# mj129/Tramba

Measured on AMD Instinct MI355X. Metric: images/sec fwd Tramba-V 384x384, higher is better.
Workload: dtype bf16; 1 GPU; Tramba-V (VMamba-B encoder) 384x384 bf16 inference, batch 4 per GPU, random-init weights (seed 1026), randn images; global_batch=4, launch=hipGraph replay, decoder guide branches on a side stream

## Files before the change

include/tramba_hip.h:

```cpp
#ifndef TRAMBA_HIP_H
#define TRAMBA_HIP_H

#include <stddef.h>
#include <stdint.h>

#ifdef __cplusplus
extern "C" {
#endif

typedef enum { TRAMBA_F32 = 0, TRAMBA_F16 = 1, TRAMBA_BF16 = 2 } tramba_dtype;

typedef enum {
    TRAMBA_SCAN_RASTER = 0,
    TRAMBA_SCAN_LINE = 1,
    TRAMBA_SCAN_HELIX = 2,
    TRAMBA_SCAN_WINDOW = 3,
    TRAMBA_SCAN_DILATION = 4
} tramba_scan_family;

typedef enum { TRAMBA_ACT_NONE = 0, TRAMBA_ACT_SILU = 1, TRAMBA_ACT_GELU = 2,
               TRAMBA_ACT_SIGMOID_GATE = 3 ,
               TRAMBA_ACT_GELU_GRAD_MUL = 4
             } tramba_act;

// ... 6 lines not shown
int tramba_abi_version(void);
int tramba_device_error(void);
int tramba_profile_enable(int which, int enable);
int tramba_profile_read(int which, double *total_ms, double *total_bytes);
int tramba_profile_min_units(int which, double min_units);
int tramba_tune_set(int knob, int value);
int tramba_tune_get(int knob);
#define TRAMBA_TUNE_MERGE_FORM 0
#define TRAMBA_TUNE_SCAN_FORM 1
#define TRAMBA_TUNE_SCAN_W 2
#define TRAMBA_TUNE_GEMM_TILE 3
#define TRAMBA_TUNE_MAILBOX_SKIP 4
#define TRAMBA_TUNE_DW_FORM 6
#define TRAMBA_TUNE_DW_ROWS 7
#define TRAMBA_TUNE_MERGE_PW 8
#define TRAMBA_TUNE_COUNT 9
#define TRAMBA_PROF_SCAN_BOUNDARY 0
#define TRAMBA_PROF_SCAN_FUSED 1
#define TRAMBA_PROF_GEMM 2
#define TRAMBA_PROF_MERGE 3
#define TRAMBA_PROF_SCAN_BWD 4
#define TRAMBA_PROF_WGRAD 5
#define TRAMBA_PROF_LAYERNORM 6
#define TRAMBA_PROF_DW 7
#define TRAMBA_PROF_COUNT 8

int tramba_scan_family_k(int family);
int tramba_default_window(int h);
int tramba_scan_table(int family, int h, int w, int param, int32_t *out);
int tramba_scan_table_inverse(const int32_t *table, int k, int l, int32_t *inv_ptr, int32_t *inv_idx);

// ... 115 lines not shown
int tramba_slab_sum(const float *part, float *out, int64_t n, int nslab, void *stream);
int tramba_multi_sum_strided(const float *const *parts, float *const *outs, const int64_t *n, const int64_t *stride,
                             const int *nslab, int count, void *stream);
int tramba_multi_sum(const float *const *parts, float *const *outs, const int64_t *n, const int *nslab, int count,
                     void *stream);

int tramba_expand_norm_head_cl(const void *x, const void *w, const float *ln_w, const float *ln_b,
                               const float *head_w, float head_b, float *y, int batch, int h, int wd, int cin, int p,
                               float eps, int dtype, void *stream);

int tramba_conv3x3s2_cl(const void *x, const void *w, const float *bias, void *y, int batch, int hin,
                        int win, int cin, int cout, int dtype, void *stream);
int tramba_stem_conv_ln_gelu(const void *img, const float *w, const float *bias, const float *ln_w,
                             const float *ln_b, void *y, int batch, int h, int wd, float eps,
                             int img_dtype, int dtype, void *stream);

#define TRAMBA_EVAL_NINT 520
#define TRAMBA_EVAL_NDBL 48
int tramba_saliency_stats(const float *pred, const unsigned char *gt, long long *ints, double *dbl, int batch, int h,
                          int w, void *stream);
#define TRAMBA_WFM_MAX_DIM 4096
int tramba_feature_transform(const unsigned char *gt, int *idx, int *dist2, int batch, int h, int w, void *stream);
size_t tramba_weighted_f_workspace(int batch, int h, int w);
int tramba_weighted_f_sums(const float *pred, const unsigned char *gt, const int *idx, const int *dist2, const double *gauss,
                           double *sums, void *workspace, size_t workspace_bytes, int batch, int h, int w, void *stream);

#define TRAMBA_FRAME_MAX_DIM 16384
#define TRAMBA_FRAME_MAX_OUT 2048
size_t tramba_resize_table_words(int in_h, int in_w, int out_h, int out_w);
int tramba_resize_table(int in_h, int in_w, int out_h, int out_w, const double *mean, const double *std, int *table,
// ... 120 lines not shown
```

tramba_amd/csrc/linear.hip:

```cpp
#include <stdlib.h>
#include <string.h>

#include <type_traits>

#include "common.h"

namespace tramba {

typedef __attribute__((ext_vector_type(8))) short frag8_t;
typedef __attribute__((ext_vector_type(8))) _Float16 frag8h_t;
typedef __attribute__((ext_vector_type(16))) float acc16_t;

template <typename T> struct Mfma;
template <> struct Mfma<__hip_bfloat16> {
    static constexpr int KSTEP = 16;
    using frag = frag8_t;
    static __device__ __forceinline__ acc16_t run(frag a, frag b, acc16_t c)
    {
        typedef __attribute__((ext_vector_type(8))) __bf16 bf8;
        return __builtin_amdgcn_mfma_f32_32x32x16_bf16(__builtin_bit_cast(bf8, a), __builtin_bit_cast(bf8, b), c, 0, 0, 0);
    }
};
template <> struct Mfma<__half> {
    static constexpr int KSTEP = 16;
// ... 567 lines not shown
    }
    for (; kt0 + NS <= nk; kt0 += NS) {
#pragma unroll
        for (int ui = 0; ui < NS; ++ui) kstep(kt0 + ui, ui & 1, pipe[ui % NS], pipe[(ui + 1) % NS]);
    }
#pragma unroll
    for (int ui = 0; ui < NS - 1; ++ui)
        if (kt0 + ui < nk) kstep(kt0 + ui, ui & 1, pipe[ui % NS], pipe[(ui + 1) % NS]);

    if constexpr (LNHEAD) {
        static_assert(BN == 128, "one tile = whole 128-channel groups");
        tile_epilogue_ln_head<T, BM>(acc, lds, hd, M, m0, n0);
    } else {
        tile_epilogue<T, TO, BM, BN>(acc, lds, bias, res, y, M, N, act, m0, n0);
    }
}

#define TRAMBA_DSR128_(OUT, ADDR, OFF) asm volatile("ds_read_b128 %0, %1 offset:" #OFF : "=v"(OUT) : "v"(ADDR) : "memory")

template <typename T, typename TO, int NSTG, bool LNIN = false, bool DUAL = false>
__global__ __launch_bounds__(256) void linear_dma_kernel(const T *__restrict__ x, const T *__restrict__ w,
                                                        const float *__restrict__ bias, const T *__restrict__ res,
                                                        TO *__restrict__ y, long M, int N, int K, int act,
                                                        LnIn li = LnIn{nullptr, 0.f}, TO *__restrict__ y_pre = nullptr)
{
#if defined(__HIP_DEVICE_COMPILE__)
    constexpr int BM = 64, BN = 64;
    constexpr int TILE_BYTES = (BM + BN) * kBK * 2;
    constexpr int EPI_BYTES = BM * (BN + 4) * 4;
    constexpr int LDS_BYTES = NSTG * TILE_BYTES > EPI_BYTES ? NSTG * TILE_BYTES : EPI_BYTES;
// ... 1041 lines not shown
extern "C" int tramba_expand_norm_head_cl(const void *x, const void *w, const float *ln_w, const float *ln_b,
                                          const float *head_w, float head_b, float *y, int batch, int h, int wd, int cin,
                                          int p, float eps, int dtype, void *stream)
{
    TRAMBA_CHECK(x && w && ln_w && ln_b && head_w && y, "expand_norm_head_cl: null tensor");
    TRAMBA_CHECK(batch > 0 && h > 0 && wd > 0 && cin > 0 && p > 0, "expand_norm_head_cl: empty shape");
    TRAMBA_CHECK(dtype == TRAMBA_BF16 || dtype == TRAMBA_F16, "expand_norm_head_cl: 16-bit dtypes only");
    TRAMBA_CHECK(cin % 64 == 0, "expand_norm_head_cl: Cin=%d must be a multiple of 64", cin);
    TRAMBA_CHECK(aligned16(x) && aligned16(w), "expand_norm_head_cl: tensors must be 16-byte aligned");
    const long m = (long)batch * h * wd;
    const int n = p * p * 128;
    TRAMBA_CHECK(m < 2147483647L && (m + 63) / 64 <= 65535, "expand_norm_head_cl: too many pixels");
    hipStream_t s = (hipStream_t)stream;
    ProfScope prof(TRAMBA_PROF_GEMM, s, 2.0 * (double)m * n * cin);
    const LnHead hd{ln_w, ln_b, head_w, head_b, eps, h, wd, p, y};
    dim3 grid((unsigned)(n / 128), (unsigned)((m + 63) / 64)), block(256);
    if (dtype == TRAMBA_BF16) {
        using T = __hip_bfloat16;
        hipLaunchKernelGGL((linear_lean_kernel<T, T, 64, 128, 1, true>), grid, block, 0, s, (const T *)x, (const T *)w,
                           (const float *)nullptr, (const T *)nullptr, (T *)nullptr, m, n, cin, 0, (const T *)nullptr, 0, hd);
    } else {
        using T = __half;
        hipLaunchKernelGGL((linear_lean_kernel<T, T, 64, 128, 1, true>), grid, block, 0, s, (const T *)x, (const T *)w,
                           (const float *)nullptr, (const T *)nullptr, (T *)nullptr, m, n, cin, 0, (const T *)nullptr, 0, hd);
    }
    TRAMBA_LAUNCH_CHECK();
    return TRAMBA_OK;
}

extern "C" int tramba_conv3x3s2_cl(const void *x, const void *w, const float *bias, void *y, int batch, int hin,
// ... 43 lines not shown
```

tramba_amd/csrc/stem.hip:

```cpp
#include "common.h"

namespace tramba {

constexpr int kStemCout = 64, kStemTaps = 27;

template <typename TI, typename T>
__global__ __launch_bounds__(256) void stem_conv_ln_gelu_kernel(const TI *__restrict__ img, const float *__restrict__ w,
                                                               const float *__restrict__ bias,
                                                               const float *__restrict__ ln_w,
                                                               const float *__restrict__ ln_b, T *__restrict__ y,
                                                               int B, int H, int W, int Ho, int Wo, float eps)
{
    __shared__ __attribute__((aligned(16))) float wl[kStemTaps][kStemCout];
    for (int t = threadIdx.x; t < kStemTaps * kStemCout; t += blockDim.x) {
        const int co = t / kStemTaps, tap = t % kStemTaps;
        wl[tap][co] = w[t];
    }
    __syncthreads();
    const long pix = (long)blockIdx.x * 64 + (threadIdx.x >> 2);
    const int part = threadIdx.x & 3;
    const long npix = (long)B * Ho * Wo;
    const bool ok = pix < npix;
    const long pp = ok ? pix : npix - 1;
    const int wo = (int)(pp % Wo);
    const long t2 = pp / Wo;
    const int ho = (int)(t2 % Ho), b = (int)(t2 / Ho);

    float acc[16];
#pragma unroll
    for (int j = 0; j < 16; ++j) acc[j] = bias[part * 16 + j];
#pragma unroll 1
    for (int ci = 0; ci < 3; ++ci)
#pragma unroll 1
        for (int ky = 0; ky < 3; ++ky) {
            const int hy = 2 * ho + ky - 1;
#pragma unroll
            for (int kx = 0; kx < 3; ++kx) {
                const int wx = 2 * wo + kx - 1;
                float v = 0.f;
                if (hy >= 0 && hy < H && wx >= 0 && wx < W) v = Cvt<TI>::to_f(img[(((long)b * 3 + ci) * H + hy) * W + wx]);
                const float4 *wp = reinterpret_cast<const float4 *>(&wl[ci * 9 + ky * 3 + kx][part * 16]);
#pragma unroll
                for (int q = 0; q < 4; ++q) {
                    const float4 ww = wp[q];
                    acc[4 * q + 0] = fmaf(v, ww.x, acc[4 * q + 0]);
                    acc[4 * q + 1] = fmaf(v, ww.y, acc[4 * q + 1]);
                    acc[4 * q + 2] = fmaf(v, ww.z, acc[4 * q + 2]);
                    acc[4 * q + 3] = fmaf(v, ww.w, acc[4 * q + 3]);
                }
            }
        }
    float s = 0.f;
#pragma unroll
    for (int j = 0; j < 16; ++j) s += acc[j];
    s += __shfl_xor(s, 1, 4);
    s += __shfl_xor(s, 2, 4);
    const float mean = s * (1.f / kStemCout);
    float q2 = 0.f;
#pragma unroll
    for (int j = 0; j < 16; ++j) {
        const float d = acc[j] - mean;
        q2 = fmaf(d, d, q2);
    }
    q2 += __shfl_xor(q2, 1, 4);
    q2 += __shfl_xor(q2, 2, 4);
    const float rstd = rsqrtf(q2 * (1.f / kStemCout) + eps);
    if (!ok) return;
    T *yo = y + pix * kStemCout + part * 16;
#pragma unroll
    for (int h8 = 0; h8 < 2; ++h8) {
        float o[8];
#pragma unroll
        for (int j = 0; j < 8; ++j) {
            const int c = part * 16 + h8 * 8 + j;
            o[j] = geluf_((acc[h8 * 8 + j] - mean) * rstd * ln_w[c] + ln_b[c]);
        }
        store_pack<T, 8>(yo + h8 * 8, o);
    }
}

}

using namespace tramba;

extern "C" int tramba_stem_conv_ln_gelu(const void *img, const float *w, const float *bias, const float *ln_w,
                                        const float *ln_b, void *y, int batch, int h, int wd, float eps,
                                        int img_dtype, int dtype, void *stream)
{
    TRAMBA_CHECK(img && w && bias && ln_w && ln_b && y, "stem_conv_ln_gelu: null tensor");
    TRAMBA_CHECK(batch > 0 && h > 0 && wd > 0, "stem_conv_ln_gelu: empty shape");
    TRAMBA_CHECK(img_dtype == TRAMBA_F32 || img_dtype == dtype, "stem_conv_ln_gelu: image must be f32 or the activation dtype");
    TRAMBA_CHECK(aligned16(y), "stem_conv_ln_gelu: output must be 16-byte aligned");
    const int ho = (h + 1) / 2, wo = (wd + 1) / 2;
    const long npix = (long)batch * ho * wo;
    dim3 grid((unsigned)((npix + 63) / 64)), block(256);
    hipStream_t s = (hipStream_t)stream;
    TRAMBA_DISPATCH_DTYPE(dtype, T, {
        if (img_dtype == TRAMBA_F32 && dtype != TRAMBA_F32)
            hipLaunchKernelGGL((stem_conv_ln_gelu_kernel<float, T>), grid, block, 0, s, (const float *)img, w, bias, ln_w,
                               ln_b, (T *)y, batch, h, wd, ho, wo, eps);
        else
            hipLaunchKernelGGL((stem_conv_ln_gelu_kernel<T, T>), grid, block, 0, s, (const T *)img, w, bias, ln_w, ln_b,
                               (T *)y, batch, h, wd, ho, wo, eps);
    });
    TRAMBA_LAUNCH_CHECK();
    return TRAMBA_OK;
}
```

tramba_amd/hip.py:

```python
import ctypes
import os
import threading
import weakref

import numpy as np
import torch

_HERE = os.path.dirname(os.path.abspath(__file__))
LIB_PATH = os.path.join(_HERE, "_lib", "libtramba_hip.so")

F32, F16, BF16 = 0, 1, 2
ACT_NONE, ACT_SILU, ACT_GELU, ACT_SIGMOID_GATE, ACT_GELU_GRAD_MUL = 0, 1, 2, 3, 4
SCAN_RASTER, SCAN_LINE, SCAN_HELIX, SCAN_WINDOW, SCAN_DILATION = range(5)
FAMILY = {"raster": SCAN_RASTER, "line": SCAN_LINE, "helix": SCAN_HELIX, "window": SCAN_WINDOW,
          "dilation": SCAN_DILATION}
PROF_SCAN_BOUNDARY, PROF_SCAN_FUSED, PROF_GEMM, PROF_MERGE, PROF_SCAN_BWD, PROF_WGRAD, PROF_LAYERNORM, PROF_DW = 0, 1, 2, 3, 4, 5, 6, 7

_DT = {torch.float32: F32, torch.float16: F16, torch.bfloat16: BF16}

c_int, c_i64, c_f, c_vp = ctypes.c_int, ctypes.c_int64, ctypes.c_float, ctypes.c_void_p

SIGNATURES = {
    "tramba_last_error": (ctypes.c_char_p, []),
    "tramba_abi_version": (c_int, []),
# ... 72 lines not shown
    "tramba_linear_ln_cl": (c_int, [c_vp] * 6 + [c_i64, c_int, c_int, c_f, c_int, c_int, c_int, c_vp]),
    "tramba_linear2_cl": (c_int, [c_vp, c_vp, c_int] + [c_vp] * 4 + [c_i64, c_int, c_int, c_int, c_int, c_int, c_vp]),
    "tramba_wgrad_workspace": (ctypes.c_size_t, [c_i64, c_int, c_int, c_int, c_int]),
    "tramba_wgrad_cl": (c_int, [c_vp] * 4 + [ctypes.c_size_t, c_i64, c_int, c_int, c_int, c_int, c_i64, c_i64, c_int, c_i64,
                                             c_i64, c_int, c_int, c_int, c_vp]),
    "tramba_rows_gemm_cl": (c_int, [c_vp] * 3 + [c_int, c_i64, c_int, c_int, c_int, c_int, c_int, c_vp]),
    "tramba_shadow_cast_multi": (c_int, [c_vp, c_int, c_i64, c_int, c_vp]),
    "tramba_slab_sum": (c_int, [c_vp, c_vp, c_i64, c_int, c_vp]),
    "tramba_multi_sum": (c_int, [c_vp, c_vp, c_vp, c_vp, c_int, c_vp]),
    "tramba_multi_sum_strided": (c_int, [c_vp, c_vp, c_vp, c_vp, c_vp, c_int, c_vp]),
    "tramba_wgrad_parts_cl": (c_int, [c_vp] * 4 + [ctypes.c_size_t, c_i64, c_int, c_int, c_int, c_int, c_i64, c_i64, c_int, c_i64,
                                                   c_i64, c_int, c_int, c_int, c_vp, c_vp]),
    "tramba_expand_norm_head_cl": (c_int, [c_vp] * 5 + [c_f, c_vp] + [c_int] * 5 + [c_f, c_int, c_vp]),
    "tramba_conv3x3s2_cl": (c_int, [c_vp] * 4 + [c_int] * 6 + [c_vp]),
    "tramba_stem_conv_ln_gelu": (c_int, [c_vp] * 6 + [c_int] * 3 + [c_f, c_int, c_int, c_vp]),
    "tramba_sod_loss_sums": (c_int, [c_vp] * 3 + [c_int] * 6 + [c_vp]),
    "tramba_sod_loss_finish": (c_int, [c_vp] * 4 + [c_int, c_int, c_i64, c_vp, c_vp]),
    "tramba_sod_loss_grad_workspace": (ctypes.c_size_t, [c_int] * 5),
    "tramba_sod_loss_grad": (c_int, [c_vp] * 6 + [ctypes.c_size_t] + [c_int] * 5 + [c_vp]),
    "tramba_loss_weight_map": (c_int, [c_vp] * 2 + [c_int] * 4 + [c_vp]),
    "tramba_sod_wloss_sums": (c_int, [c_vp] * 4 + [c_int] * 6 + [c_f, c_int, c_vp]),
    "tramba_sod_wloss_finish": (c_int, [c_vp] * 4 + [c_int, c_int, c_i64, c_int, c_int, c_vp, c_vp]),
    "tramba_sod_wloss_grad_workspace": (ctypes.c_size_t, [c_int] * 5),
    "tramba_sod_wloss_grad": (c_int, [c_vp] * 7 + [ctypes.c_size_t] + [c_int] * 5 + [c_f, c_int, c_vp]),
    "tramba_adam_step": (c_int, [c_vp] * 6 + [c_int] + [ctypes.c_double] * 5 + [c_vp]),
    "tramba_grad_accumulate": (c_int, [c_vp] * 3 + [c_int, c_vp, c_vp]),
    "tramba_grad_norm_workspace": (ctypes.c_size_t, [c_vp, c_int]),
    "tramba_grad_norm": (c_int, [c_vp] * 2 + [c_int, ctypes.c_double, ctypes.c_double, c_int, c_vp, c_vp, ctypes.c_size_t, c_vp]),
    "tramba_adam_step_ctl": (c_int, [c_vp] * 6 + [c_int] + [ctypes.c_double] * 5 + [c_vp] * 3),
    "tramba_window_attn_cl": (c_int, [c_vp] * 3 + [c_int] * 8 + [c_vp]),
# ... 144 lines not shown
        self.inv_idx = torch.from_numpy(idx).to(device)
        if not torch.cuda.is_current_stream_capturing():
            torch.cuda.current_stream(device).synchronize()


def scan_order(family: str, h: int, w: int, device, param: int = 0) -> ScanOrder:
    key = (family, h, w, param, str(device))
    so = _table_cache.get(key)
    if so is None:
        so = _table_cache[key] = ScanOrder(family, h, w, param, device)
    return so


TUNE_MERGE_FORM, TUNE_SCAN_FORM, TUNE_SCAN_W, TUNE_GEMM_TILE, TUNE_MAILBOX_SKIP, TUNE_DW_FORM, TUNE_DW_ROWS = 0, 1, 2, 3, 4, 6, 7
TUNE_MERGE_PW = 8


def device_error():
    _check(lib().tramba_device_error(), "device_error")


def tune_set(knob: int, value: int):
    _check(lib().tramba_tune_set(knob, value), "tune_set")


def profile_enable(which: int, on: bool):
    _check(lib().tramba_profile_enable(which, int(on)), "profile_enable")


def profile_min_units(which: int, min_units: float):
# ... 1297 lines not shown
    _check(lib().tramba_shadow_cast_multi(_ptr(table), ntensors, total_tiles, _DT[dtype], _stream()), "shadow_cast_multi")


def conv3x3s2_cl(x, w_kmajor, bias):
    _dev(x, w_kmajor, bias)
    bb, h, wd, cin = x.shape
    cout = w_kmajor.shape[0]
    if w_kmajor.dtype != x.dtype or w_kmajor.shape[1] != 9 * cin:
        raise TrambaHipError("conv3x3s2_cl: weight dtype/shape mismatch")
    y = torch.empty((bb, (h + 1) // 2, (wd + 1) // 2, cout), dtype=x.dtype, device=x.device)
    _check(lib().tramba_conv3x3s2_cl(_ptr(x), _ptr(w_kmajor), _ptr(bias), _ptr(y), bb, h, wd, cin, cout, dt(x),
                                     _stream()), "conv3x3s2_cl")
    return y


def stem_conv_ln_gelu(img, w, bias, ln_w, ln_b, eps, out_dtype):
    _dev(img, w, bias, ln_w, ln_b)
    bb, c3, h, wd = img.shape
    if c3 != 3 or tuple(w.shape) != (64, 3, 3, 3):
        raise TrambaHipError("stem_conv_ln_gelu: expects a 3 -> 64 channel 3x3 stem")
    y = torch.empty((bb, (h + 1) // 2, (wd + 1) // 2, 64), dtype=out_dtype, device=img.device)
    _check(lib().tramba_stem_conv_ln_gelu(_ptr(img), _ptr(w), _ptr(bias), _ptr(ln_w), _ptr(ln_b), _ptr(y), bb, h, wd,
                                          eps, _DT[img.dtype], _DT[out_dtype], _stream()), "stem_conv_ln_gelu")
    return y


_PATCH_EMBED_FORMS = ((7, 4, 3, 64), (4, 4, 0, 128))


def patch_conv_supported(dtype, cin, cout, r):
    return dtype in _ATTN_DTYPES and 2 <= r <= 8 and cin > 0 and cin % 64 == 0 and cout > 0 and cout % 8 == 0


def patch_conv_cl(x, w_kmajor, bias):
    _dev(x, w_kmajor, bias)
    if x.dim() != 4 or w_kmajor.dim() != 4 or w_kmajor.dtype != x.dtype or w_kmajor.shape[1] != w_kmajor.shape[2] \
# ... 306 lines not shown
```

tramba_amd/models.py:

```python
from collections import OrderedDict

import torch
import torch.nn as nn
import torch.nn.functional as F

from . import hip
from .modules import (FinalPatchExpand_X4, FreqBlockv6, LayerNorm2d, Linear2d, MultiScaleDecoderBlock, PatchExpand,
                      VSSMEncoder, _cache, _infer, _init_weights, _run_blocks, model_mask_pool, _need_device, from_cl,
                      load_pretrained_Base, to_cl)
from .ops import CrossMerge_Line, CrossScan_Line


OVERLAP_BRANCHES = True
OVERLAP_TRAINING = True
_side_streams = {}


def _side_stream(device):
    key = str(device)
    st = _side_streams.get(key)
    if st is None:
        st = _side_streams[key] = torch.cuda.Stream(device=device)
    return st

# ... 10 lines not shown
        if g is not None and g.is_cuda:
            here = torch.cuda.current_stream(g.device)
            if here != ctx.consumer:
                ev = torch.cuda.Event()
                ev.record(here)
                ctx.consumer.wait_event(ev)
            g.record_stream(ctx.consumer)
            if _DEBUG_STREAMS is not None:
                _DEBUG_STREAMS.append((here.cuda_stream, ctx.consumer.cuda_stream))
        return g, None


_DEBUG_STREAMS = None
_OVERLAP_TRAINING_STAGES = None
_OVERLAP_INFER_STAGES = None


def _bias_scalar(conv: nn.Conv2d) -> float:
    b = conv.bias
    if b is None:
        return 0.0
    key = (b._version, b.data_ptr())
    hit = conv.__dict__.get("_tramba_bias_scalar")
    if hit is None or hit[0] != key:
        hit = conv.__dict__["_tramba_bias_scalar"] = (key, float(b.detach().float().item()))
    return hit[1]


class VSSMDecoder(nn.Module):

# ... 96 lines not shown

    def forward(self, skips):
        return self._forward_cl([skips[0]] + [to_cl(s) for s in skips[1:]])


class BaseUMamba(nn.Module):

    def __init__(self, vss_args, decoder_args, use_pretrain=True, pretrained_path=""):
        super().__init__()
        self.vssm_encoder = VSSMEncoder(**vss_args)
        self.decoder = VSSMDecoder(**decoder_args)
        self.compute_dtype = None
        if use_pretrain:
            load_pretrained_Base(self.vssm_encoder, ckpt_path=pretrained_path)

    def _forward_overlapped(self, x):
        main = torch.cuda.current_stream()
        side = _side_stream(x.device)
        dec = self.decoder
        n = len(dec.stage_layers)
        guides = {}

        def on_stage(i, feat):
            s = n - 2 - i
            if s < 0 or s >= len(dec.guide_layers):
                return
            if (torch.is_grad_enabled() and _OVERLAP_TRAINING_STAGES is not None and s not in _OVERLAP_TRAINING_STAGES) or (
                    not torch.is_grad_enabled() and _OVERLAP_INFER_STAGES is not None and s not in _OVERLAP_INFER_STAGES):
                return
            side.wait_stream(main)
            feat.record_stream(side)
            with torch.cuda.stream(side):
                fin = _StreamEdge.apply(feat, main) if torch.is_grad_enabled() and feat.requires_grad else feat
                mid = dec.guide_layers[s]._forward_cl(fin)
                ready = torch.cuda.Event()
                ready.record(side)
            guides[s] = (mid, ready)

        skips = self.vssm_encoder._forward_cl(x, on_stage=on_stage)
        out = dec._forward_cl(skips, guides=guides)
        main.wait_stream(side)
        return out

    def forward(self, x):
        _need_device(x)
        if self.training:
            model_mask_pool(self).begin_step()
        if self.compute_dtype is not None:
            x = x.to(self.compute_dtype)
        if OVERLAP_BRANCHES and (OVERLAP_TRAINING or not torch.is_grad_enabled()) and type(self.decoder) is VSSMDecoder:
            out = self._forward_overlapped(x)
        else:
            skips = self.vssm_encoder._forward_cl(x)
            out = self.decoder._forward_cl(skips)
        if self.compute_dtype is not None:
            out = [o.float() for o in out] if isinstance(out, list) else out.float()
        return out

    @torch.no_grad()
    def freeze_encoder(self):
        for name, p in self.vssm_encoder.named_parameters():
            if "patch_embed" not in name:
                p.requires_grad = False

    @torch.no_grad()
    def unfreeze_encoder(self):
        for p in self.vssm_encoder.parameters():
            p.requires_grad = True
# ... 282 lines not shown
```

tramba_amd/modules.py:

```python
import math
from collections import OrderedDict

import torch
import torch.nn as nn
import torch.nn.functional as F

from . import hip
from .ops import (CrossMerge, CrossMerge_Dilation, CrossMerge_Line, CrossMerge_Window, CrossScan,
                  CrossScan_Dilation, CrossScan_Line, CrossScan_Window, SelectiveScanOflex)



FOLD_LAYERNORM = True


def to_cl(x: torch.Tensor) -> torch.Tensor:
    return x.permute(0, 2, 3, 1).contiguous()


def from_cl(x: torch.Tensor) -> torch.Tensor:
    return x.permute(0, 3, 1, 2)


def _need_device(x):
# ... 1720 lines not shown
            nn.Identity(), LayerNorm2d(dims[0]))
        self.layers = nn.ModuleList()
        self.downsample = nn.ModuleList()
        for i in range(self.num_layers):
            if i < self.num_layers - 1:
                self.downsample.append(nn.Sequential(
                    nn.Identity(), nn.Conv2d(dims[i], dims[i] * 2, kernel_size=3, stride=2, padding=1),
                    nn.Identity(), LayerNorm2d(dims[i] * 2)))
            else:
                self.downsample.append(nn.Identity())
            blocks = [VSSBlock(hidden_dim=dims[i], drop_path=dp, norm_layer=LayerNorm2d, channel_first=True)
                      for dp in dpr[sum(depths[:i]):sum(depths[:i + 1])]]
            self.layers.append(nn.Sequential(OrderedDict(blocks=nn.Sequential(*blocks))))
        self.apply(_init_weights)

    def _forward_cl(self, x_img, on_stage=None):
        feats = [x_img]
        pe = self.patch_embed
        if (_infer(x_img, pe[0].weight) and pe[0].in_channels == 3 and pe[0].out_channels == 64
                and pe[0].kernel_size == (3, 3) and pe[0].stride == (2, 2) and x_img.is_contiguous()):
            act_dtype = pe[5].weight.dtype if pe[5].weight.dtype != torch.float32 else x_img.dtype
            x = hip.stem_conv_ln_gelu(x_img, _f32(pe[0].weight), _f32(pe[0].bias), _f32(pe[2].weight),
                                      _f32(pe[2].bias), pe[2].eps, act_dtype)
        else:
            x = _conv_cl(pe[0], to_cl(x_img))
            x = pe[2]._forward_cl(x, act=hip.ACT_GELU)
        x = _conv_cl(pe[5], x)
        x = pe[7]._forward_cl(x)
        for s, layer in enumerate(self.layers):
            x = _run_blocks(layer.blocks, x)
            feats.append(x)
            if on_stage is not None:
                on_stage(s, x)
            if s < self.num_layers - 1:
                ds = self.downsample[s]
                x = ds[3]._forward_cl(_conv_cl(ds[1], x))
        return feats

    def forward(self, x):
# ... 34 lines not shown
```

Measured before the change: 883.1 img/s.

## Add row-panel expand head kernel, tile stem conv via LDS, fold input cast

Adds a new kernel for the final expand+LayerNorm+head. It keeps each row block's activations in registers and streams the 128x128 weight panels of each pixel-shuffle group through double-buffered LDS, which replaces the previous per-group GEMM tiling. The stem conv kernel is rewritten to stage a 2D image patch and the weights in LDS, and each thread now computes several output pixels instead of doing redundant global image loads. The fp32-to-bf16 input cast is folded into the stem kernel, which rounds the input in registers, removing a separate cast pass over the image. Together these change two end-of-pipeline kernels plus the model wrapper, and add new tuning knobs.

```diff
diff --git a/include/tramba_hip.h b/include/tramba_hip.h
--- a/include/tramba_hip.h
+++ b/include/tramba_hip.h
@@ -44,7 +44,9 @@
 #define TRAMBA_TUNE_DW_FORM 6
 #define TRAMBA_TUNE_DW_ROWS 7
 #define TRAMBA_TUNE_MERGE_PW 8
-#define TRAMBA_TUNE_COUNT 9
+#define TRAMBA_TUNE_HEAD_FORM 9
+#define TRAMBA_TUNE_STEM_PIXELS 10
+#define TRAMBA_TUNE_COUNT 11
 #define TRAMBA_PROF_SCAN_BOUNDARY 0
 #define TRAMBA_PROF_SCAN_FUSED 1
 #define TRAMBA_PROF_GEMM 2
@@ -190,6 +192,9 @@
 int tramba_stem_conv_ln_gelu(const void *img, const float *w, const float *bias, const float *ln_w,
                              const float *ln_b, void *y, int batch, int h, int wd, float eps,
                              int img_dtype, int dtype, void *stream);
+int tramba_stem_conv_ln_gelu_r(const void *img, const float *w, const float *bias, const float *ln_w,
+                               const float *ln_b, void *y, int batch, int h, int wd, float eps,
+                               int img_dtype, int dtype, int round_input, void *stream);
 
 #define TRAMBA_EVAL_NINT 520
 #define TRAMBA_EVAL_NDBL 48
diff --git a/tramba_amd/csrc/linear.hip b/tramba_amd/csrc/linear.hip
--- a/tramba_amd/csrc/linear.hip
+++ b/tramba_amd/csrc/linear.hip
@@ -605,6 +605,153 @@
     } else {
         tile_epilogue<T, TO, BM, BN>(acc, lds, bias, res, y, M, N, act, m0, n0);
     }
+}
+
+constexpr int kHeadBM = 128, kHeadC = 128;
+constexpr int kHeadPanelBytes = kHeadC * kHeadC * 2;
+
+template <typename T>
+__global__ __launch_bounds__(256, 2) void expand_head_rows_kernel(const T *__restrict__ x, const T *__restrict__ w, long M, int G,
+                                                                 int gper, LnHead hd)
+{
+#if defined(__HIP_DEVICE_COMPILE__)
+    constexpr int K = kHeadC;
+    __shared__ __attribute__((aligned(1024))) unsigned char panel[2 * kHeadPanelBytes];
+    __shared__ __attribute__((aligned(16))) float prm[3][kHeadC];
+    const int tid = threadIdx.x, lane = tid & 63, wave = tid >> 6;
+    const int r32 = lane & 31, hi = lane >> 5;
+    const long m0 = (long)blockIdx.y * kHeadBM;
+    const int g0 = blockIdx.x * gper;
+    const int g1 = g0 + gper < G ? g0 + gper : G;
+    const long mrows = M - m0 < kHeadBM ? M - m0 : kHeadBM;
+    const __amdgpu_buffer_rsrc_t ra = make_rsrc(x + m0 * K, (unsigned)mrows * (K * 2u));
+    const __amdgpu_buffer_rsrc_t rb = make_rsrc(w, (unsigned)G * (unsigned)kHeadPanelBytes);
+
+    v4u_t stage[8];
+    auto pload = [&](int g) {
+#pragma unroll
+        for (int i = 0; i < 8; ++i)
+            stage[i] = __builtin_amdgcn_raw_buffer_load_b128(rb, (unsigned)(tid + 256 * i) * 16u, (unsigned)g * (unsigned)kHeadPanelBytes, 0);
+    };
+    auto pstore = [&](int par) {
+        unsigned char *base = panel + par * kHeadPanelBytes;
+#pragma unroll
+        for (int i = 0; i < 8; ++i) {
+            const int q = tid + 256 * i, row = q >> 4, c16 = q & 15;
+            *reinterpret_cast<v4u_t *>(base + (c16 >> 3) * (kHeadC * 128) + row * 128 + swz_chunk(row, c16 & 7) * 16) = stage[i];
+        }
+    };
+    v4u_t afr[K / 16];
+#pragma unroll
+    for (int kk = 0; kk < K / 16; ++kk)
+        afr[kk] = __builtin_amdgcn_raw_buffer_load_b128(ra, (unsigned)(wave * 32 + r32) * (K * 2u) + (unsigned)(kk * 32 + hi * 16), 0, 0);
+    pload(g0);
+    if (tid < kHeadC) {
+        prm[0][tid] = hd.ln_w[tid];
+        prm[1][tid] = hd.ln_b[tid];
+        prm[2][tid] = hd.head_w[tid];
+    }
+    pstore(0);
+    __syncthreads();
+
+    const long grow = m0 + wave * 32 + r32;
+    const bool rowok = hi == 0 && grow < M;
+    long obase = 0;
+    {
+        const unsigned pix = (unsigned)(rowok ? grow : 0);
+        const unsigned wi = pix % (unsigned)hd.W, bh = pix / (unsigned)hd.W;
+        const unsigned hh = bh % (unsigned)hd.H, bb = bh / (unsigned)hd.H;
+        obase = ((long)bb * (hd.H * hd.P) + (long)hh * hd.P) * (long)(hd.W * hd.P) + (long)wi * hd.P;
+    }
+    const unsigned lbase = (unsigned)(size_t)(__attribute__((address_space(3))) unsigned char *)panel;
+    unsigned brd[4];
+#pragma unroll
+    for (int j = 0; j < 4; ++j) {
+        const int row = j * 32 + r32;
+        brd[j] = (unsigned)(row * 128 + swz_chunk(row, hi) * 16);
+    }
+
+    for (int g = g0; g < g1; ++g) {
+        const int par = (g - g0) & 1;
+        if (g + 1 < g1) pload(g + 1);
+        acc16_t acc[4];
+#pragma unroll
+        for (int j = 0; j < 4; ++j)
+#pragma unroll
+            for (int r = 0; r < 16; ++r) acc[j][r] = 0.f;
+        frag8_t b[2][4];
+        const unsigned pb = lbase + (unsigned)(par * kHeadPanelBytes);
+#define TRAMBA_HEAD_RD_(KK)                                                                                                           \
+    do {                                                                                                                             \
+        _Pragma("unroll") for (int j = 0; j < 4; ++j) {                                                                              \
+            const unsigned ad = pb + (brd[j] ^ (unsigned)(((KK) & 3) * 32));                                                         \
+            if ((KK) < 4) asm volatile("ds_read_b128 %0, %1" : "=v"(b[(KK) & 1][j]) : "v"(ad) : "memory");                             \
+            else asm volatile("ds_read_b128 %0, %1 offset:16384" : "=v"(b[(KK) & 1][j]) : "v"(ad) : "memory");                         \
+        }                                                                                                                            \
+    } while (0)
+        TRAMBA_HEAD_RD_(0);
+#pragma unroll
+        for (int kk = 0; kk < K / 16; ++kk) {
+            frag8_t(&bk)[4] = b[kk & 1];
+            if (kk + 1 < K / 16) {
+                TRAMBA_HEAD_RD_(kk + 1);
+                asm volatile("s_waitcnt lgkmcnt(4)" : "+v"(bk[0]), "+v"(bk[1]), "+v"(bk[2]), "+v"(bk[3]) : : "memory");
+            } else {
+                asm volatile("s_waitcnt lgkmcnt(0)" : "+v"(bk[0]), "+v"(bk[1]), "+v"(bk[2]), "+v"(bk[3]) : : "memory");
+            }
+#pragma unroll
+            for (int j = 0; j < 4; ++j)
+                acc[j] = Mfma<T>::run(bk[j], __builtin_bit_cast(frag8_t, afr[kk]), acc[j]);
+        }
+#undef TRAMBA_HEAD_RD_
+        auto join8 = [](const float (&p)[8]) { return ((p[0] + p[1]) + (p[2] + p[3])) + ((p[4] + p[5]) + (p[6] + p[7])); };
+        float p1[8];
+#pragma unroll
+        for (int c = 0; c < 8; ++c) p1[c] = acc[0][c];
+#pragma unroll
+        for (int t = 1; t < 8; ++t)
+#pragma unroll
+            for (int c = 0; c < 8; ++c) p1[c] += acc[t >> 1][8 * (t & 1) + c];
+        float s1 = join8(p1);
+        s1 += __shfl_xor(s1, 32, 64);
+        const float mean = s1 * (1.f / 128.f);
+        float p2[8];
+#pragma unroll
+        for (int t = 0; t < 8; ++t)
+#pragma unroll
+            for (int c = 0; c < 8; ++c) {
+                const float d = acc[t >> 1][8 * (t & 1) + c] - mean;
+                p2[c] = t == 0 ? d * d : fmaf(d, d, p2[c]);
+            }
+        float s2 = join8(p2);
+        s2 += __shfl_xor(s2, 32, 64);
+        const float rstd = rsqrtf(s2 * (1.f / 128.f) + hd.eps);
+        float pd[8];
+#pragma unroll
+        for (int t = 0; t < 8; ++t) {
+            const int j = t >> 1;
+#pragma unroll
+            for (int qq = 0; qq < 2; ++qq) {
+                const int q = 2 * (t & 1) + qq;
+                const int ch = 32 * j + 8 * q + 4 * hi;
+                const float4 ga = *reinterpret_cast<const float4 *>(&prm[0][ch]);
+                const float4 be = *reinterpret_cast<const float4 *>(&prm[1][ch]);
+                const float4 hw = *reinterpret_cast<const float4 *>(&prm[2][ch]);
+                const float gav[4] = {ga.x, ga.y, ga.z, ga.w}, bev[4] = {be.x, be.y, be.z, be.w}, hwv[4] = {hw.x, hw.y, hw.z, hw.w};
+#pragma unroll
+                for (int e = 0; e < 4; ++e) {
+                    const float yn = (acc[j][4 * q + e] - mean) * rstd * gav[e] + bev[e];
+                    pd[4 * qq + e] = t == 0 ? yn * hwv[e] : fmaf(yn, hwv[e], pd[4 * qq + e]);
+                }
+            }
+        }
+        float dot = join8(pd);
+        dot += __shfl_xor(dot, 32, 64);
+        if (rowok) hd.out[obase + (long)(g / hd.P) * (long)(hd.W * hd.P) + (g % hd.P)] = dot + hd.head_b;
+        if (g + 1 < g1) pstore(par ^ 1);
+        __syncthreads();
+    }
+#endif
 }
 
 #define TRAMBA_DSR128_(OUT, ADDR, OFF) asm volatile("ds_read_b128 %0, %1 offset:" #OFF : "=v"(OUT) : "v"(ADDR) : "memory")
@@ -1676,6 +1823,24 @@
     hipStream_t s = (hipStream_t)stream;
     ProfScope prof(TRAMBA_PROF_GEMM, s, 2.0 * (double)m * n * cin);
     const LnHead hd{ln_w, ln_b, head_w, head_b, eps, h, wd, p, y};
+    const int form = tramba_tune_get(TRAMBA_TUNE_HEAD_FORM);
+    TRAMBA_CHECK(form == 0 || form == 1 || (form > 100 && form <= 100 + 64), "TRAMBA_TUNE_HEAD_FORM %d: 0, 1 or 101..164", form);
+    if (cin == kHeadC && form != 1 && (long)p * p * kHeadPanelBytes < 2147483648L) {
+        const int groups = p * p;
+        const long mt = (m + kHeadBM - 1) / kHeadBM;
+        int gper = groups;
+        while (gper > 1 && mt * ((groups + gper - 1) / gper) < 4 * 256) gper = (gper + 1) / 2;
+        if (form > 100) gper = form - 100 < groups ? form - 100 : groups;
+        dim3 grid((unsigned)((groups + gper - 1) / gper), (unsigned)mt), block(256);
+        if (dtype == TRAMBA_BF16)
+            hipLaunchKernelGGL((expand_head_rows_kernel<__hip_bfloat16>), grid, block, 0, s, (const __hip_bfloat16 *)x,
+                               (const __hip_bfloat16 *)w, m, groups, gper, hd);
+        else
+            hipLaunchKernelGGL((expand_head_rows_kernel<__half>), grid, block, 0, s, (const __half *)x, (const __half *)w, m,
+                               groups, gper, hd);
+        TRAMBA_LAUNCH_CHECK();
+        return TRAMBA_OK;
+    }
     dim3 grid((unsigned)(n / 128), (unsigned)((m + 63) / 64)), block(256);
     if (dtype == TRAMBA_BF16) {
         using T = __hip_bfloat16;
diff --git a/tramba_amd/csrc/stem.hip b/tramba_amd/csrc/stem.hip
--- a/tramba_amd/csrc/stem.hip
+++ b/tramba_amd/csrc/stem.hip
@@ -3,106 +3,188 @@
 namespace tramba {
 
 constexpr int kStemCout = 64, kStemTaps = 27;
+constexpr int kStemTH = 4;
+constexpr int kStemPR = 2 * kStemTH + 1;
+constexpr int kStemThreads = kStemTH * 64;
 
-template <typename TI, typename T>
-__global__ __launch_bounds__(256) void stem_conv_ln_gelu_kernel(const TI *__restrict__ img, const float *__restrict__ w,
-                                                               const float *__restrict__ bias,
-                                                               const float *__restrict__ ln_w,
-                                                               const float *__restrict__ ln_b, T *__restrict__ y,
-                                                               int B, int H, int W, int Ho, int Wo, float eps)
+template <typename TI, typename T, int NP>
+__global__ __launch_bounds__(kStemThreads) void stem_conv_ln_gelu_kernel(const TI *__restrict__ img, const float *__restrict__ w,
+                                                                        const float *__restrict__ bias,
+                                                                        const float *__restrict__ ln_w,
+                                                                        const float *__restrict__ ln_b, T *__restrict__ y,
+                                                                        int B, int H, int W, int Ho, int Wo, int tiles_w,
+                                                                        int tiles_h, float eps, int round_input)
 {
+    constexpr int TW = 16 * NP, PC = 2 * TW + 1, PLD = 2 * TW + 4;
     __shared__ __attribute__((aligned(16))) float wl[kStemTaps][kStemCout];
-    for (int t = threadIdx.x; t < kStemTaps * kStemCout; t += blockDim.x) {
-        const int co = t / kStemTaps, tap = t % kStemTaps;
-        wl[tap][co] = w[t];
+    __shared__ float patch[3 * kStemPR][PLD];
+    const int tid = threadIdx.x;
+    const int tw = (int)(blockIdx.x % (unsigned)tiles_w);
+    const unsigned t1 = blockIdx.x / (unsigned)tiles_w;
+    const int th = (int)(t1 % (unsigned)tiles_h), b = (int)(t1 / (unsigned)tiles_h);
+    const int ho0 = th * kStemTH, wo0 = tw * TW;
+    const int hy0 = 2 * ho0 - 1, wx0 = 2 * wo0 - 1;
+
+    {
+        constexpr int kPPerT = (3 * kStemPR * PC + kStemThreads - 1) / kStemThreads;
+        constexpr int kWPerT = (kStemTaps * kStemCout + kStemThreads - 1) / kStemThreads;
+        float pv[kPPerT], wv[kWPerT];
+#pragma unroll
+        for (int i = 0; i < kPPerT; ++i) {
+            const int e = tid + i * kStemThreads, r = e / PC, c = e % PC;
+            const int ci = r / kStemPR, hy = hy0 + r % kStemPR, wx = wx0 + c;
+            const bool ok = r < 3 * kStemPR && hy >= 0 && hy < H && wx >= 0 && wx < W;
+            pv[i] = ok ? Cvt<TI>::to_f(img[(((long)b * 3 + ci) * H + hy) * W + wx]) : 0.f;
+        }
+#pragma unroll
+        for (int i = 0; i < kWPerT; ++i) {
+            const int t = tid + i * kStemThreads;
+            wv[i] = t < kStemTaps * kStemCout ? w[t] : 0.f;
+        }
+#pragma unroll
+        for (int i = 0; i < kPPerT; ++i) {
+            const int e = tid + i * kStemThreads, r = e / PC, c = e % PC;
+            if (r < 3 * kStemPR) patch[r][c] = round_input ? Cvt<T>::to_f(Cvt<T>::from_f(pv[i])) : pv[i];
+        }
+#pragma unroll
+        for (int i = 0; i < kWPerT; ++i) {
+            const int t = tid + i * kStemThreads;
+            const int co = t / kStemTaps, tap = t % kStemTaps;
+            if (t < kStemTaps * kStemCout) wl[tap][co] = wv[i];
+        }
     }
     __syncthreads();
-    const long pix = (long)blockIdx.x * 64 + (threadIdx.x >> 2);
-    const int part = threadIdx.x & 3;
-    const long npix = (long)B * Ho * Wo;
-    const bool ok = pix < npix;
-    const long pp = ok ? pix : npix - 1;
-    const int wo = (int)(pp % Wo);
-    const long t2 = pp / Wo;
-    const int ho = (int)(t2 % Ho), b = (int)(t2 / Ho);
 
-    float acc[16];
+    const int part = tid & 3;
+    const int pc = (tid >> 2) & 15;
+    const int pr = tid >> 6;
+    const int ho = ho0 + pr;
+
+    float acc[NP][16];
 #pragma unroll
-    for (int j = 0; j < 16; ++j) acc[j] = bias[part * 16 + j];
+    for (int j = 0; j < 16; ++j) {
+        const float bj = bias[part * 16 + j];
+#pragma unroll
+        for (int p = 0; p < NP; ++p) acc[p][j] = bj;
+    }
 #pragma unroll 1
     for (int ci = 0; ci < 3; ++ci)
 #pragma unroll 1
         for (int ky = 0; ky < 3; ++ky) {
-            const int hy = 2 * ho + ky - 1;
+            const float *prow = &patch[ci * kStemPR + 2 * pr + ky][2 * pc];
 #pragma unroll
             for (int kx = 0; kx < 3; ++kx) {
-                const int wx = 2 * wo + kx - 1;
-                float v = 0.f;
-                if (hy >= 0 && hy < H && wx >= 0 && wx < W) v = Cvt<TI>::to_f(img[(((long)b * 3 + ci) * H + hy) * W + wx]);
+                float v[NP];
+#pragma unroll
+                for (int p = 0; p < NP; ++p) v[p] = prow[32 * p + kx];
                 const float4 *wp = reinterpret_cast<const float4 *>(&wl[ci * 9 + ky * 3 + kx][part * 16]);
 #pragma unroll
                 for (int q = 0; q < 4; ++q) {
                     const float4 ww = wp[q];
-                    acc[4 * q + 0] = fmaf(v, ww.x, acc[4 * q + 0]);
-                    acc[4 * q + 1] = fmaf(v, ww.y, acc[4 * q + 1]);
-                    acc[4 * q + 2] = fmaf(v, ww.z, acc[4 * q + 2]);
-                    acc[4 * q + 3] = fmaf(v, ww.w, acc[4 * q + 3]);
+#pragma unroll
+                    for (int p = 0; p < NP; ++p) {
+                        acc[p][4 * q + 0] = fmaf(v[p], ww.x, acc[p][4 * q + 0]);
+                        acc[p][4 * q + 1] = fmaf(v[p], ww.y, acc[p][4 * q + 1]);
+                        acc[p][4 * q + 2] = fmaf(v[p], ww.z, acc[p][4 * q + 2]);
+                        acc[p][4 * q + 3] = fmaf(v[p], ww.w, acc[p][4 * q + 3]);
+                    }
                 }
             }
         }
-    float s = 0.f;
-#pragma unroll
-    for (int j = 0; j < 16; ++j) s += acc[j];
-    s += __shfl_xor(s, 1, 4);
-    s += __shfl_xor(s, 2, 4);
-    const float mean = s * (1.f / kStemCout);
-    float q2 = 0.f;
+    float gam[16], bet[16];
 #pragma unroll
     for (int j = 0; j < 16; ++j) {
-        const float d = acc[j] - mean;
-        q2 = fmaf(d, d, q2);
+        gam[j] = ln_w[part * 16 + j];
+        bet[j] = ln_b[part * 16 + j];
     }
-    q2 += __shfl_xor(q2, 1, 4);
-    q2 += __shfl_xor(q2, 2, 4);
-    const float rstd = rsqrtf(q2 * (1.f / kStemCout) + eps);
-    if (!ok) return;
-    T *yo = y + pix * kStemCout + part * 16;
 #pragma unroll
-    for (int h8 = 0; h8 < 2; ++h8) {
-        float o[8];
+    for (int p = 0; p < NP; ++p) {
+        float s = 0.f;
 #pragma unroll
-        for (int j = 0; j < 8; ++j) {
-            const int c = part * 16 + h8 * 8 + j;
-            o[j] = geluf_((acc[h8 * 8 + j] - mean) * rstd * ln_w[c] + ln_b[c]);
+        for (int j = 0; j < 16; ++j) s += acc[p][j];
+        s += __shfl_xor(s, 1, 4);
+        s += __shfl_xor(s, 2, 4);
+        const float mean = s * (1.f / kStemCout);
+        float q2 = 0.f;
+#pragma unroll
+        for (int j = 0; j < 16; ++j) {
+            const float d = acc[p][j] - mean;
+            q2 = fmaf(d, d, q2);
         }
-        store_pack<T, 8>(yo + h8 * 8, o);
+        q2 += __shfl_xor(q2, 1, 4);
+        q2 += __shfl_xor(q2, 2, 4);
+        const float rstd = rsqrtf(q2 * (1.f / kStemCout) + eps);
+        const int wo = wo0 + 16 * p + pc;
+        if (ho < Ho && wo < Wo) {
+            T *yo = y + (((long)b * Ho + ho) * Wo + wo) * kStemCout + part * 16;
+#pragma unroll
+            for (int h8 = 0; h8 < 2; ++h8) {
+                float o[8];
+#pragma unroll
+                for (int j = 0; j < 8; ++j)
+                    o[j] = geluf_((acc[p][h8 * 8 + j] - mean) * rstd * gam[h8 * 8 + j] + bet[h8 * 8 + j]);
+                store_pack<T, 8>(yo + h8 * 8, o);
+            }
+        }
     }
+}
+
+template <typename TI, typename T, int NP>
+static void launch_stem(const void *img, const float *w, const float *bias, const float *ln_w, const float *ln_b, void *y,
+                        int batch, int h, int wd, int ho, int wo, float eps, int round_input, hipStream_t s)
+{
+    const int tiles_w = (wo + 16 * NP - 1) / (16 * NP), tiles_h = (ho + kStemTH - 1) / kStemTH;
+    dim3 grid((unsigned)((long)batch * tiles_h * tiles_w)), block(kStemThreads);
+    hipLaunchKernelGGL((stem_conv_ln_gelu_kernel<TI, T, NP>), grid, block, 0, s, (const TI *)img, w, bias, ln_w, ln_b, (T *)y,
+                       batch, h, wd, ho, wo, tiles_w, tiles_h, eps, round_input);
+}
+
+static int stem_pixels_per_thread(long npix)
+{
+    const int forced = tramba_tune_get(TRAMBA_TUNE_STEM_PIXELS);
+    if (forced) return forced;
+    for (int np = 4; np > 1; np /= 2)
+        if (npix >= 4L * 1024 * 16 * np) return np;
+    return 1;
 }
 
 }
 
 using namespace tramba;
 
+extern "C" int tramba_stem_conv_ln_gelu_r(const void *img, const float *w, const float *bias, const float *ln_w,
+                                          const float *ln_b, void *y, int batch, int h, int wd, float eps,
+                                          int img_dtype, int dtype, int round_input, void *stream)
+{
+    TRAMBA_CHECK(img && w && bias && ln_w && ln_b && y, "stem_conv_ln_gelu: null tensor");
+    TRAMBA_CHECK(batch > 0 && h > 0 && wd > 0, "stem_conv_ln_gelu: empty shape");
+    TRAMBA_CHECK(img_dtype == TRAMBA_F32 || img_dtype == dtype, "stem_conv_ln_gelu: image must be f32 or the activation dtype");
+    TRAMBA_CHECK(round_input == 0 || round_input == 1, "stem_conv_ln_gelu: round_input must be 0 or 1");
+    TRAMBA_CHECK(aligned16(y), "stem_conv_ln_gelu: output must be 16-byte aligned");
+    const int ho = (h + 1) / 2, wo = (wd + 1) / 2;
+    TRAMBA_CHECK((long)batch * ((ho + kStemTH - 1) / kStemTH) * ((wo + 15) / 16) < 2147483647L, "stem_conv_ln_gelu: too many output tiles");
+    const int forced = tramba_tune_get(TRAMBA_TUNE_STEM_PIXELS);
+    TRAMBA_CHECK(forced == 0 || forced == 1 || forced == 2 || forced == 4, "TRAMBA_TUNE_STEM_PIXELS %d: 0, 1, 2 or 4", forced);
+    const int np = stem_pixels_per_thread((long)batch * ho * wo);
+    hipStream_t s = (hipStream_t)stream;
+#define TRAMBA_STEM_(TI_, T_, RI_)                                                                                                   \
+    do {                                                                                                                             \
+        if (np == 4) launch_stem<TI_, T_, 4>(img, w, bias, ln_w, ln_b, y, batch, h, wd, ho, wo, eps, RI_, s);                        \
+        else if (np == 2) launch_stem<TI_, T_, 2>(img, w, bias, ln_w, ln_b, y, batch, h, wd, ho, wo, eps, RI_, s);                   \
+        else launch_stem<TI_, T_, 1>(img, w, bias, ln_w, ln_b, y, batch, h, wd, ho, wo, eps, RI_, s);                                \
+    } while (0)
+    TRAMBA_DISPATCH_DTYPE(dtype, T, {
+        if (img_dtype == TRAMBA_F32 && dtype != TRAMBA_F32) TRAMBA_STEM_(float, T, round_input);
+        else TRAMBA_STEM_(T, T, 0);
+    });
+#undef TRAMBA_STEM_
+    TRAMBA_LAUNCH_CHECK();
+    return TRAMBA_OK;
+}
+
 extern "C" int tramba_stem_conv_ln_gelu(const void *img, const float *w, const float *bias, const float *ln_w,
                                         const float *ln_b, void *y, int batch, int h, int wd, float eps,
                                         int img_dtype, int dtype, void *stream)
 {
-    TRAMBA_CHECK(img && w && bias && ln_w && ln_b && y, "stem_conv_ln_gelu: null tensor");
-    TRAMBA_CHECK(batch > 0 && h > 0 && wd > 0, "stem_conv_ln_gelu: empty shape");
-    TRAMBA_CHECK(img_dtype == TRAMBA_F32 || img_dtype == dtype, "stem_conv_ln_gelu: image must be f32 or the activation dtype");
-    TRAMBA_CHECK(aligned16(y), "stem_conv_ln_gelu: output must be 16-byte aligned");
-    const int ho = (h + 1) / 2, wo = (wd + 1) / 2;
-    const long npix = (long)batch * ho * wo;
-    dim3 grid((unsigned)((npix + 63) / 64)), block(256);
-    hipStream_t s = (hipStream_t)stream;
-    TRAMBA_DISPATCH_DTYPE(dtype, T, {
-        if (img_dtype == TRAMBA_F32 && dtype != TRAMBA_F32)
-            hipLaunchKernelGGL((stem_conv_ln_gelu_kernel<float, T>), grid, block, 0, s, (const float *)img, w, bias, ln_w,
-                               ln_b, (T *)y, batch, h, wd, ho, wo, eps);
-        else
-            hipLaunchKernelGGL((stem_conv_ln_gelu_kernel<T, T>), grid, block, 0, s, (const T *)img, w, bias, ln_w, ln_b,
-                               (T *)y, batch, h, wd, ho, wo, eps);
-    });
-    TRAMBA_LAUNCH_CHECK();
-    return TRAMBA_OK;
+    return tramba_stem_conv_ln_gelu_r(img, w, bias, ln_w, ln_b, y, batch, h, wd, eps, img_dtype, dtype, 0, stream);
 }
diff --git a/tramba_amd/hip.py b/tramba_amd/hip.py
--- a/tramba_amd/hip.py
+++ b/tramba_amd/hip.py
@@ -110,6 +110,7 @@
     "tramba_expand_norm_head_cl": (c_int, [c_vp] * 5 + [c_f, c_vp] + [c_int] * 5 + [c_f, c_int, c_vp]),
     "tramba_conv3x3s2_cl": (c_int, [c_vp] * 4 + [c_int] * 6 + [c_vp]),
     "tramba_stem_conv_ln_gelu": (c_int, [c_vp] * 6 + [c_int] * 3 + [c_f, c_int, c_int, c_vp]),
+    "tramba_stem_conv_ln_gelu_r": (c_int, [c_vp] * 6 + [c_int] * 3 + [c_f, c_int, c_int, c_int, c_vp]),
     "tramba_sod_loss_sums": (c_int, [c_vp] * 3 + [c_int] * 6 + [c_vp]),
     "tramba_sod_loss_finish": (c_int, [c_vp] * 4 + [c_int, c_int, c_i64, c_vp, c_vp]),
     "tramba_sod_loss_grad_workspace": (ctypes.c_size_t, [c_int] * 5),
@@ -284,6 +285,7 @@
 
 TUNE_MERGE_FORM, TUNE_SCAN_FORM, TUNE_SCAN_W, TUNE_GEMM_TILE, TUNE_MAILBOX_SKIP, TUNE_DW_FORM, TUNE_DW_ROWS = 0, 1, 2, 3, 4, 6, 7
 TUNE_MERGE_PW = 8
+TUNE_HEAD_FORM, TUNE_STEM_PIXELS = 9, 10
 
 
 def device_error():
@@ -1611,12 +1613,16 @@
     return y
 
 
-def stem_conv_ln_gelu(img, w, bias, ln_w, ln_b, eps, out_dtype):
+def stem_conv_ln_gelu(img, w, bias, ln_w, ln_b, eps, out_dtype, round_input=False):
     _dev(img, w, bias, ln_w, ln_b)
     bb, c3, h, wd = img.shape
     if c3 != 3 or tuple(w.shape) != (64, 3, 3, 3):
         raise TrambaHipError("stem_conv_ln_gelu: expects a 3 -> 64 channel 3x3 stem")
     y = torch.empty((bb, (h + 1) // 2, (wd + 1) // 2, 64), dtype=out_dtype, device=img.device)
+    if round_input:
+        _check(lib().tramba_stem_conv_ln_gelu_r(_ptr(img), _ptr(w), _ptr(bias), _ptr(ln_w), _ptr(ln_b), _ptr(y), bb, h, wd,
+                                                eps, _DT[img.dtype], _DT[out_dtype], 1, _stream()), "stem_conv_ln_gelu")
+        return y
     _check(lib().tramba_stem_conv_ln_gelu(_ptr(img), _ptr(w), _ptr(bias), _ptr(ln_w), _ptr(ln_b), _ptr(y), bb, h, wd,
                                           eps, _DT[img.dtype], _DT[out_dtype], _stream()), "stem_conv_ln_gelu")
     return y
diff --git a/tramba_amd/models.py b/tramba_amd/models.py
--- a/tramba_amd/models.py
+++ b/tramba_amd/models.py
@@ -48,6 +48,7 @@
 _DEBUG_STREAMS = None
 _OVERLAP_TRAINING_STAGES = None
 _OVERLAP_INFER_STAGES = None
+_FOLD_INPUT_CAST = True
 
 
 def _bias_scalar(conv: nn.Conv2d) -> float:
@@ -174,7 +175,7 @@
         if use_pretrain:
             load_pretrained_Base(self.vssm_encoder, ckpt_path=pretrained_path)
 
-    def _forward_overlapped(self, x):
+    def _forward_overlapped(self, x, round_input=False):
         main = torch.cuda.current_stream()
         side = _side_stream(x.device)
         dec = self.decoder
@@ -197,7 +198,7 @@
                 ready.record(side)
             guides[s] = (mid, ready)
 
-        skips = self.vssm_encoder._forward_cl(x, on_stage=on_stage)
+        skips = self.vssm_encoder._forward_cl(x, on_stage=on_stage, round_input=round_input)
         out = dec._forward_cl(skips, guides=guides)
         main.wait_stream(side)
         return out
@@ -206,12 +207,15 @@
         _need_device(x)
         if self.training:
             model_mask_pool(self).begin_step()
-        if self.compute_dtype is not None:
+        fold = (_FOLD_INPUT_CAST and self.compute_dtype in (torch.bfloat16, torch.float16) and x.dtype == torch.float32
+                and type(self.vssm_encoder) is VSSMEncoder and self.vssm_encoder._fused_stem(x)
+                and self.vssm_encoder.patch_embed[5].weight.dtype == self.compute_dtype)
+        if self.compute_dtype is not None and not fold:
             x = x.to(self.compute_dtype)
         if OVERLAP_BRANCHES and (OVERLAP_TRAINING or not torch.is_grad_enabled()) and type(self.decoder) is VSSMDecoder:
-            out = self._forward_overlapped(x)
+            out = self._forward_overlapped(x, round_input=fold)
         else:
-            skips = self.vssm_encoder._forward_cl(x)
+            skips = self.vssm_encoder._forward_cl(x, round_input=fold)
             out = self.decoder._forward_cl(skips)
         if self.compute_dtype is not None:
             out = [o.float() for o in out] if isinstance(out, list) else out.float()
diff --git a/tramba_amd/modules.py b/tramba_amd/modules.py
--- a/tramba_amd/modules.py
+++ b/tramba_amd/modules.py
@@ -1758,15 +1758,20 @@
             self.layers.append(nn.Sequential(OrderedDict(blocks=nn.Sequential(*blocks))))
         self.apply(_init_weights)
 
-    def _forward_cl(self, x_img, on_stage=None):
+    def _fused_stem(self, x_img) -> bool:
+        pe = self.patch_embed
+        return (_infer(x_img, pe[0].weight) and pe[0].in_channels == 3 and pe[0].out_channels == 64
+                and pe[0].kernel_size == (3, 3) and pe[0].stride == (2, 2) and x_img.is_contiguous())
+
+    def _forward_cl(self, x_img, on_stage=None, round_input=False):
         feats = [x_img]
         pe = self.patch_embed
-        if (_infer(x_img, pe[0].weight) and pe[0].in_channels == 3 and pe[0].out_channels == 64
-                and pe[0].kernel_size == (3, 3) and pe[0].stride == (2, 2) and x_img.is_contiguous()):
+        if self._fused_stem(x_img):
             act_dtype = pe[5].weight.dtype if pe[5].weight.dtype != torch.float32 else x_img.dtype
             x = hip.stem_conv_ln_gelu(x_img, _f32(pe[0].weight), _f32(pe[0].bias), _f32(pe[2].weight),
-                                      _f32(pe[2].bias), pe[2].eps, act_dtype)
+                                      _f32(pe[2].bias), pe[2].eps, act_dtype, round_input=round_input)
         else:
+            assert not round_input, "round_input is the fused stem's argument"
             x = _conv_cl(pe[0], to_cl(x_img))
             x = pe[2]._forward_cl(x, act=hip.ACT_GELU)
         x = _conv_cl(pe[5], x)
```

New measurement: 889.1 img/s, median of 5. Within noise of the previous version (+0.7%).
